# NJUVISION/PCGCv2

Hardware: AMD Instinct MI355X
Metric: encode+decode Mpoints/sec at fixed bpp (r3 ckpt), vox10 frame (higher is better)
Workload: dtype f32

## Files before the change

pcgcv2_amd/csrc/child_irn.hip:

```cpp
#include "child_kernels.h"

#define DECL_IRN_LAUNCH(NAME) int NAME(const int32_t* parent_nbr, int64_t n_parent, const float* in, int in_ld, const float* table, \
                                       int table_bytes, const IrnEpi& ep, hipStream_t s)
DECL_IRN_LAUNCH(pcgc_irn_child_a16); DECL_IRN_LAUNCH(pcgc_irn_child_b16);
DECL_IRN_LAUNCH(pcgc_irn_child_a32); DECL_IRN_LAUNCH(pcgc_irn_child_b32);

extern "C" int pcgc_irn_child_pass(const int32_t* parent_nbr, int64_t n_parent, int C, int pass, const float* in, int in_ld,
                                   const float* table, int64_t table_bytes, const float* b0, const float* b1, const float* b2,
                                   const float* x, int x_ld, float* out, int out_ld, void* stream) {
    CHILD_COMMON_CHECKS(in_ld)
    PCGC_REQUIRE(C == 16 || C == 32, "channels must be 16 or 32 (C = 64 blocks run on pcgc_irn_rows_pass through the level's own map)");
    PCGC_REQUIRE(pass == 1 || pass == 2, "pass must be 1 (A) or 2 (B)");
    PCGC_REQUIRE(out && b0 && b1 && (pass == 1 || (b2 && x)), "null argument");
    PCGC_REQUIRE((out_ld & 3) == 0 && (((uintptr_t)out) & 15) == 0 && (pass == 1 || ((x_ld & 3) == 0 && (((uintptr_t)x) & 15) == 0)),
                 "rows must be 16-byte aligned");
    PCGC_REQUIRE(pass == 2 || out_ld == C / 2, "pass A writes a dense [rows, C/2] tensor");
    hipStream_t s = S(stream);
    IrnEpi ep{b0, b1, b2, x, x_ld, out, out_ld};
    const int tb = (int)table_bytes;
    int rc;
    if (pass == 1) {
        PCGC_REQUIRE(table_bytes == (int64_t)(C == 16 ? 52 : 38) * (C / 16) * 1024, "pass A table size");
        rc = C == 16 ? pcgc_irn_child_a16(parent_nbr, n_parent, in, in_ld, table, tb, ep, s) : pcgc_irn_child_a32(parent_nbr, n_parent, in, in_ld, table, tb, ep, s);
    } else {
        PCGC_REQUIRE(table_bytes == (int64_t)(C == 16 ? 85 * 64 * 4 : 64 * 128 * 4), "pass B table size");
        rc = C == 16 ? pcgc_irn_child_b16(parent_nbr, n_parent, in, in_ld, table, tb, ep, s) : pcgc_irn_child_b32(parent_nbr, n_parent, in, in_ld, table, tb, ep, s);
    }
    if (rc) return rc;
    PCGC_CHECK_LAUNCH("irn_child_pass");
    return 0;
}

#ifdef PCGC_CHILD_TIMING
extern "C" int pcgc_child_timing_irn(unsigned long long* out8, int reset) {
    hipDeviceSynchronize();
    if (out8) hipMemcpyFromSymbol(out8, HIP_SYMBOL(g_child_dbg), 8 * sizeof(unsigned long long));
    if (reset) { unsigned long long z[8] = {0}; hipMemcpyToSymbol(HIP_SYMBOL(g_child_dbg), z, sizeof(z)); }
    return 0;
}
// ... 2 lines not shown
```

pcgcv2_amd/csrc/child_kernels.h:

```cpp
#pragma once
#include "pcgc_common.h"
#include "mfma_util.h"
#include <type_traits>

#ifdef PCGC_CHILD_TIMING
static __device__ unsigned long long g_child_dbg[8];
#define CHILD_T(var) const unsigned long long var = __builtin_amdgcn_s_memtime()
#define CHILD_TADD(slot, a, b) do { child_dbg[slot] += (b) - (a); } while (0)
#define CHILD_DBG_DECL unsigned long long child_dbg[8] = {0, 0, 0, 0, 0, 0, 0, 0};
#define CHILD_DBG_PARAM , unsigned long long (&child_dbg)[8]
#define CHILD_DBG_ARG , child_dbg
#define CHILD_TFLUSH do { if ((threadIdx.x & 63) == 0) { for (int q_ = 0; q_ < 8; ++q_) if (child_dbg[q_]) atomicAdd(&g_child_dbg[q_], child_dbg[q_]); } } while (0)
#define CHILD_TIMING_READER(NAME)                                                                                      \
    extern "C" int NAME(unsigned long long* out8, int reset) {                                                         \
        (void)hipDeviceSynchronize();                                                                                  \
        if (out8) (void)hipMemcpyFromSymbol(out8, HIP_SYMBOL(g_child_dbg), 8 * sizeof(unsigned long long));           \
        if (reset) { unsigned long long z[8] = {0}; (void)hipMemcpyToSymbol(HIP_SYMBOL(g_child_dbg), z, sizeof(z)); }  \
        return 0;                                                                                                      \
    }
#else
#define CHILD_T(var)
#define CHILD_TADD(slot, a, b)
#define CHILD_DBG_DECL
#define CHILD_DBG_PARAM
// ... 86 lines not shown
    static constexpr int tz(int t) { return CPT == 4 ? (t % TH) : (t % TH) >> 1; }
    static constexpr int ty(int t) { return (t % TH) & 1; }
    static constexpr bool active(int c, int t) {
        const int kz = cz_of(c) - tz(t);
        if (HZ >= 0 && tz(t) != HZ) return false;
        if (CPT == 4) {
            if (t < TH) return in02(kz);
            return kz == 1 && (cy_of(c) == 1 || cy_of(c) == 2) && (cx_of(c) == 1 || cx_of(c) == 2);
        }
        const int ky = cy_of(c) - ty(t);
        if (t < TH) return in02(kz) && in02(ky);
        return kz == 1 && ky == 1 && (cx_of(c) == 1 || cx_of(c) == 2);
    }
    static constexpr int N0 = CPT == 4 ? 48 : (CPT == 2 ? 36 : 27);
    static constexpr int frag(int c, int t) {
        const int kz = cz_of(c) - tz(t);
        if (CPT == 4) return t < TH ? kz * 16 + (c & 15) : N0 + (cy_of(c) - 1) * 2 + (cx_of(c) - 1);
        const int ky = cy_of(c) - ty(t);
        return t < TH ? (kz * 3 + ky) * 4 + cx_of(c) : N0 + (cx_of(c) - 1);
    }
    static constexpr bool uses_block(int, int) { return true; }
    static constexpr int frag_off(int c, int t, int cb) { return (frag(c, t) * NB + cb) * 64 * KS * 4; }
};
template <int C, int HZ = -1, bool T2_ = false>
struct PassB : HaloGeometry {
    static constexpr bool T2 = T2_;
    static_assert(!T2_ || C == 16, "the split layout exists for C = 16");
    static constexpr int Q = C / 4, NB = 1, ROWCHUNKS = Q / 2 , KS = Q / 4;
    static constexpr int CPT0 = 16 / (2 * Q) , T0 = 8 / CPT0, CPT1 = 16 / Q, T1 = 8 / CPT1, T = T0 + T1;
    static constexpr int Z_HALF = HZ;
    static_assert(HZ < 0 || CPT1 <= 2, "half units: no tile may hold children of both z halves");
    static constexpr bool HALF = false;
    static constexpr int kfirst(int t) { return t < T0 ? 0 : KS; }
    static constexpr int tile_z(int t) { return t < T0 ? ((t * CPT0) >> 2) & 1 : (((t - T0) * CPT1) >> 2) & 1; }
    static constexpr bool active(int c, int t) {
        if (HZ >= 0 && tile_z(t) != HZ) return false;
        if (t < T0) {
            if (CPT0 == 1) return (cell_reach(c) >> t) & 1;
            return in02(cz_of(c) - (t >> 1)) && in02(cy_of(c) - (t & 1));
        }
        const int u = t - T0;
        if (CPT1 == 2) return in02(cz_of(c) - (u >> 1)) && in02(cy_of(c) - (u & 1));
        return in02(cz_of(c) - u);
    }
    static constexpr int N0 = CPT0 == 1 ? 27 : 36;
    static constexpr int N1 = CPT1 == 2 ? 36 : 48;
    static constexpr int FRAG_W12 = N0 + N1;
    static constexpr int frag(int c, int t) {
        if (t < T0) {
            if (CPT0 == 1) return cell_k(c, t);
            return ((cz_of(c) - (t >> 1)) * 3 + (cy_of(c) - (t & 1))) * 4 + cx_of(c);
        }
        const int u = t - T0;
        if (CPT1 == 2) return N0 + ((cz_of(c) - (u >> 1)) * 3 + (cy_of(c) - (u & 1))) * 4 + cx_of(c);
        return N0 + (cz_of(c) - u) * 16 + (c & 15);
    }
    static constexpr bool uses_block(int, int) { return true; }
    static constexpr int frag_off(int c, int t, int cb) { return (frag(c, t) * NB + cb) * 64 * KS * 4; }
};

template <class V, class = void> struct child_t2_layout : std::false_type {};
template <class V> struct child_t2_layout<V, std::enable_if_t<V::T2>> : std::true_type {};

template <int I, int N, typename F>
__device__ __forceinline__ void static_for(F&& f) {
    if constexpr (I < N) {
        f(std::integral_constant<int, I>{});
        static_for<I + 1, N>(f);
    }
}

template <int KS> struct BFrag;
template <> struct BFrag<4> {
    f32x4 v;
    template <int OFF> __device__ __forceinline__ void load(unsigned base) { asm volatile("ds_read_b128 %0, %1 offset:%2" : "=v"(v) : "v"(base), "n"(OFF) : "memory"); }
    __device__ __forceinline__ void tie() { asm volatile("" : "+v"(v)); }
    __device__ __forceinline__ float get(int i) const { return v[i]; }
};
typedef float f32x2 __attribute__((ext_vector_type(2)));
template <> struct BFrag<2> {
    f32x2 v;
    template <int OFF> __device__ __forceinline__ void load(unsigned base) { asm volatile("ds_read_b64 %0, %1 offset:%2" : "=v"(v) : "v"(base), "n"(OFF) : "memory"); }
    __device__ __forceinline__ void tie() { asm volatile("" : "+v"(v)); }
    __device__ __forceinline__ float get(int i) const { return v[i]; }
};
template <> struct BFrag<1> {
// ... 27 lines not shown
    const int64_t l = (blockIdx.x >> 3) + (int64_t)(gridDim.x >> 3) * (wave + NW * i);
    const int64_t tile = (blockIdx.x & 7) * S + l;
    return (l < S && tile < ntiles) ? tile : -1;
}

template <int NW>
__device__ __forceinline__ void child_stage_table(const float* __restrict__ table, int table_bytes, unsigned char* lds_raw) {
    float4* tab = (float4*)lds_raw;
    for (int i = threadIdx.x; i < table_bytes / 16; i += NW * 64) tab[i] = ((const float4*)table)[i];
    __syncthreads();
}

struct ChildCells { int n; int c[64]; };
template <class V> constexpr ChildCells child_cells() {
    ChildCells L{};
    for (int c = 0; c < V::NCELLS; ++c) {
        bool used = false;
        for (int t = 0; t < V::T; ++t) used = used || V::active(c, t);
        if (used) L.c[L.n++] = c;
    }
    return L;
}

template <class V, int D, int MT>
__device__ __forceinline__ void child_tile_mainloop_mt(const int32_t* __restrict__ pnbr, int64_t n_p, int64_t p0,
                                                       const __amdgpu_buffer_rsrc_t& rs_in, int in_ld, const unsigned char* lds_raw,
                                                       float4* ring, f32x4 (&acc)[MT][V::T] CHILD_DBG_PARAM) {
    constexpr int NB = V::NB, T = V::T, KS = V::KS;
    static_assert(MT == 1 || MT == 2, "one or two M tiles per wave");
    static_assert((D & (D - 1)) == 0, "ring depth must be a power of two");
    static_assert((D - 1) * NB * MT < 64, "vmcnt is 6 bits");
    CHILD_T(t_tile0);
    const int lane = threadIdx.x & 63;
    const int mi = lane & 15, mq = lane >> 4;
    const int dma_r = lane >> 2;
    bool row_ok[MT];
#pragma unroll
    for (int m = 0; m < MT; ++m) row_ok[m] = p0 + 16 * m + dma_r < n_p;
    constexpr unsigned ABSENT = 0xF0000000u;
    unsigned rowb[MT][V::NMAP];
#pragma unroll
    for (int m = 0; m < MT; ++m)
#pragma unroll
        for (int kp = 0; kp < V::NMAP; ++kp) rowb[m][kp] = (unsigned)pnbr[(int64_t)kp * n_p + (row_ok[m] ? p0 + 16 * m + dma_r : 0)];
    const int f_a = (0x78 >> (2 * (mi >> 2))) & 3;
    const int dma_chunk = (lane & 3) ^ ((0x78 >> (2 * ((dma_r >> 2) & 3))) & 3);
    const bool chunk_ok = dma_chunk < V::ROWCHUNKS;
    const unsigned row_bytes = (unsigned)in_ld * 4u;
    asm volatile("s_waitcnt vmcnt(0)" ::: "memory");
#pragma unroll
    for (int m = 0; m < MT; ++m)
#pragma unroll
        for (int kp = 0; kp < V::NMAP; ++kp)
            rowb[m][kp] = (row_ok[m] && (int)rowb[m][kp] >= 0) ? rowb[m][kp] * ((unsigned)V::ROW_MUL * row_bytes) : ABSENT;
    constexpr bool T2 = child_t2_layout<V>::value;
    const unsigned lane_off = chunk_ok ? (unsigned)dma_chunk * (T2 ? 64u : 16u) : ABSENT;
    CHILD_T(t_loop0);

    constexpr ChildCells CL = child_cells<V>();
    constexpr int NC = CL.n;
    auto issue = [&](auto ii) {
        constexpr int i = decltype(ii)::value, c = CL.c[i];
        float4* dst = ring + (i & (D - 1)) * (MT * NB * 64);
#pragma unroll
        for (int m = 0; m < MT; ++m) {
            unsigned voff = rowb[m][V::kp(c)] + (T2 ? (unsigned)((V::child(c) >> 2) * 128 + (V::child(c) & 3) * 16) : (unsigned)V::child(c) * row_bytes) + lane_off +
                            (unsigned)V::byte_off(c);
            if constexpr (V::ROWCHUNKS < 4) voff = chunk_ok ? voff : 0xFFFFFFF0u;
#pragma unroll
            for (int cb = 0; cb < NB; ++cb)
                __builtin_amdgcn_raw_ptr_buffer_load_lds(rs_in, (lds_void_ptr)(dst + (m * NB + cb) * 64), 16, (int)(voff + cb * 64), 0, 0, 0);
        }
        asm volatile("" ::: "memory");
    };

#pragma unroll
    for (int m = 0; m < MT; ++m)
#pragma unroll
        for (int t = 0; t < T; ++t) acc[m][t] = (f32x4){0.f, 0.f, 0.f, 0.f};
    unsigned tab_lane;
    if constexpr (V::HALF) tab_lane = (unsigned)(uintptr_t)(lds_void_ptr)(lds_raw + V::lane_table_off(mi, mq));
    else tab_lane = (unsigned)(uintptr_t)(lds_void_ptr)((const float*)lds_raw + lane * KS);
    unsigned a_addr[4];
#pragma unroll
    for (int jj = 0; jj < 4; ++jj) a_addr[jj] = (unsigned)(uintptr_t)(lds_void_ptr)((const float*)ring + (mi * 4 + (jj ^ f_a)) * 4 + mq);
    constexpr unsigned ksteps_used = [] { unsigned m = 0; for (int t = 0; t < T; ++t) for (int j = 0; j < KS; ++j) m |= 1u << (V::kfirst(t) + j); return m; }();

    static_assert(NB * T <= 32, "all B fragments of a cell are held in registers at once");
    static_for<0, (D < NC ? D : NC)>(issue);
    static_for<0, NC>([&](auto ii) {
        constexpr int i = decltype(ii)::value, c = CL.c[i];
        constexpr int younger = (NC - 1 - i) < (D - 1) ? (NC - 1 - i) : (D - 1);
        wait_vmcnt<younger * NB * MT>();
        float a[MT][NB][4];
        BFrag<KS> b[NB][T];
        static_for<0, NB>([&](auto icb) {
            constexpr int cb = decltype(icb)::value;
            static_for<0, MT>([&](auto im) {
                constexpr int m = decltype(im)::value;
                static_for<0, 4>([&](auto ij) {
                    constexpr int jj = decltype(ij)::value;
                    if constexpr ((ksteps_used >> jj) & 1)
                        a[m][cb][jj] = lds_ld32_off<(((i & (D - 1)) * MT + m) * NB + cb) * 1024>(a_addr[jj]);
                });
            });
            static_for<0, T>([&](auto it) {
                constexpr int t = decltype(it)::value;
                if constexpr (V::active(c, t) && V::uses_block(t, cb)) {
                    constexpr int off = V::frag_off(c, t, cb);
                    if constexpr (off < 65536) b[cb][t].template load<off>(tab_lane);
                    else b[cb][t].template load<off - 65536>(tab_lane + 65536);
                }
            });
        });
        asm volatile("s_waitcnt lgkmcnt(0)" ::: "memory");
        static_for<0, NB>([&](auto icb) {
            constexpr int cb = decltype(icb)::value;
            static_for<0, MT>([&](auto im) {
                static_for<0, 4>([&](auto ij) {
                    constexpr int jj = decltype(ij)::value;
                    if constexpr ((ksteps_used >> jj) & 1) lds_tie(a[decltype(im)::value][cb][jj]);
                });
            });
            static_for<0, T>([&](auto it) {
                constexpr int t = decltype(it)::value;
                if constexpr (V::active(c, t) && V::uses_block(t, cb)) b[cb][t].tie();
            });
        });
        if constexpr (i + D < NC) issue(std::integral_constant<int, i + D>{});
        static_for<0, NB>([&](auto icb) {
            constexpr int cb = decltype(icb)::value;
            static_for<0, 4>([&](auto ij) {
                constexpr int jj = decltype(ij)::value;
                static_for<0, T>([&](auto it) {
                    constexpr int t = decltype(it)::value;
                    if constexpr (V::active(c, t) && V::uses_block(t, cb) && jj >= V::kfirst(t) && jj < V::kfirst(t) + KS) {
                        static_for<0, MT>([&](auto im) {
                            constexpr int m = decltype(im)::value;
                            acc[m][t] = __builtin_amdgcn_mfma_f32_16x16x4f32(a[m][cb][jj], b[cb][t].get(jj - V::kfirst(t)), acc[m][t], 0, 0, 0);
                        });
                    }
                });
            });
        });
    });
#ifdef PCGC_CHILD_TIMING
    asm volatile("s_nop 0" : "+v"(acc[0][0]));
    CHILD_T(t_loop1);
    CHILD_TADD(0, t_tile0, t_loop0);
    CHILD_TADD(1, t_loop0, t_loop1);
    CHILD_TADD(3, 0ull, 1ull);
#endif
}

template <class V, int D>
__device__ __forceinline__ void child_tile_mainloop(const int32_t* __restrict__ pnbr, int64_t n_p, int64_t p0,
                                                    const __amdgpu_buffer_rsrc_t& rs_in, int in_ld, const unsigned char* lds_raw,
                                                    float4* ring, f32x4 (&acc)[V::T] CHILD_DBG_PARAM) {
    child_tile_mainloop_mt<V, D, 1>(pnbr, n_p, p0, rs_in, in_ld, lds_raw, ring, reinterpret_cast<f32x4 (&)[1][V::T]>(acc) CHILD_DBG_ARG);
}

__device__ __forceinline__ void wave_lds_sync() {
    __builtin_amdgcn_fence(__ATOMIC_RELEASE, "wavefront");
    __builtin_amdgcn_wave_barrier();
    __builtin_amdgcn_fence(__ATOMIC_ACQUIRE, "wavefront");
}

template <int W, int ROWS>
struct ChildResidual { float4 x[(ROWS * (W / 4) + 63) / 64]; };
template <int W, int ROWS>
__device__ __forceinline__ void child_flush_prefetch(ChildResidual<W, ROWS>& rr, int64_t row0, int64_t rows_total, const float* __restrict__ res,
                                                     int res_ld, int lane, int half = -1) {
    constexpr int C4 = W / 4, N = (ROWS * C4 + 63) / 64;
    if (!res) return;
#pragma unroll
    for (int it = 0; it < N; ++it) {
        const int i = lane + 64 * it, lr = i / C4, c4 = i % C4;
        const int64_t row = row0 + lr;
        const bool ok = i < ROWS * C4 && row < rows_total && !(half >= 0 && ((lr >> 2) & 1) != half);
        rr.x[it] = ok ? *(const float4*)(res + row * res_ld + 4 * c4) : make_float4(0.f, 0.f, 0.f, 0.f);
    }
}
template <int W, int ROWS>
__device__ __forceinline__ void child_flush(const float* scratch, const ChildResidual<W, ROWS>& rr, bool has_res, int64_t row0, int64_t rows_total,
                                            float* __restrict__ out, int out_ld, int relu, int lane, int half = -1) {
    constexpr int C4 = W / 4, N = (ROWS * C4 + 63) / 64;
    ChildResidual<W, ROWS> xr = rr;
    if (has_res) {
#pragma unroll
        for (int it = 0; it < N; ++it) asm volatile("" : "+v"(xr.x[it].x), "+v"(xr.x[it].y), "+v"(xr.x[it].z), "+v"(xr.x[it].w));
    }
#pragma unroll
    for (int it = 0; it < N; ++it) {
        const int i = lane + 64 * it, lr = i / C4, c4 = i % C4;
        const int64_t row = row0 + lr;
        if (i >= ROWS * C4 || row >= rows_total || (half >= 0 && ((lr >> 2) & 1) != half)) continue;
        float4 v = ((const float4*)scratch)[i];
        if (has_res) {
            const float4 x = xr.x[it];
            v.x = v.x + x.x; v.y = v.y + x.y; v.z = v.z + x.z; v.w = v.w + x.w;
        }
        if (relu) { v.x = fmaxf(v.x, 0.0f); v.y = fmaxf(v.y, 0.0f); v.z = fmaxf(v.z, 0.0f); v.w = fmaxf(v.w, 0.0f); }
        *(float4*)(out + row * out_ld + 4 * c4) = v;
// ... 182 lines not shown
                child_flush<W, CH>(scratch, 8 * p0 + h * CH, 8 * n_p, ep.out, W, 0, lane, HZ);
                wave_lds_sync();
            }
        }
    };
    const int64_t nunits = (SPLIT ? 2 : 1) * ((n_p + 16 * MT - 1) / (16 * MT));
    for (int i = 0;; ++i) {
        const int64_t u = child_tile<NW>(i, wave, nunits);
        if (u < 0) break;
        CHILD_T(t_it0);
        if constexpr (SPLIT) {
            if (u & 1) unit(child_type_tag<PassA<C, 1>>{}, (u >> 1) * (16 * MT));
            else unit(child_type_tag<PassA<C, 0>>{}, (u >> 1) * (16 * MT));
        } else {
            unit(child_type_tag<V>{}, u * (16 * MT));
        }
#ifdef PCGC_CHILD_TIMING
        { CHILD_T(t_dr0); asm volatile("s_waitcnt vmcnt(0)" ::: "memory"); CHILD_T(t_it1); CHILD_TADD(5, t_dr0, t_it1); CHILD_TADD(4, t_it0, t_it1); }
#endif
    }
    CHILD_TFLUSH;
}

template <int C, int NW, int D, bool SPLIT = false, int MT = 1, bool T2 = false>
__global__ void __launch_bounds__(NW * 64)
k_child_irn_b(const int32_t* __restrict__ pnbr, int64_t n_p, const float* __restrict__ in , int in_ld,
              const float* __restrict__ table, int table_bytes, IrnEpi ep) {
    using V = PassB<C, -1, T2>;
    constexpr int Q = V::Q, H = 2 * Q, KQ = Q / 4, T0 = V::T0, T1 = V::T1, CPT0 = V::CPT0, CPT1 = V::CPT1;
    constexpr int CH = ((128 * Q + 64 * C) * 4 <= D * 1024 * MT) ? 64 : 32, MQC = CH / 32;
    constexpr int NEEDF4 = (128 * Q + CH * C) / 4;
    constexpr int RINGF4 = (D * 64 * MT > NEEDF4) ? D * 64 * MT : NEEDF4;
    CHILD_KERNEL_PROLOGUE(V, NW, D, RINGF4)
    float* us = (float*)ring;
    float* stage = us + 128 * Q;
    float w12[KQ];
#pragma unroll
    for (int jj = 0; jj < KQ; ++jj) w12[jj] = ((const float*)lds_raw)[V::FRAG_W12 * frag_floats<V>() + lane * KQ + jj];
    const int c1 = mi % Q, sub1 = mi / Q, c0 = mi % H, sub0 = mi / H;
    const float b11 = ep.b1[c1], b01 = ep.b0[c0], b12 = mi < H ? ep.b2[mi] : 0.0f;
    auto unit = [&](auto tag, const int64_t pu) {
        using VV = typename decltype(tag)::type;
        constexpr int HZ = VV::Z_HALF;
        f32x4 acc[MT][VV::T];
        child_tile_mainloop_mt<VV, D, MT>(pnbr, n_p, pu, rs_in, in_ld, lds_raw, ring, acc CHILD_DBG_ARG);
#pragma unroll
        for (int m = 0; m < MT; ++m) {
        const int64_t p0 = pu + 16 * m;
        if (m > 0 && p0 >= n_p) break;
        ChildResidual<C, CH> rr;
        child_flush_prefetch<C, CH>(rr, 8 * p0, 8 * n_p, ep.x, ep.x_ld, lane, HZ);
        {
#pragma unroll
            for (int u = 0; u < T1; ++u) {
                if (HZ >= 0 && VV::tile_z(T0 + u) != HZ) continue;
#pragma unroll
                for (int r = 0; r < 4; ++r) us[(8 * (4 * mq + r) + u * CPT1 + sub1) * Q + c1] = fmaxf(acc[m][T0 + u][r] + b11, 0.0f);
            }
        }
        wave_lds_sync();
        {
#pragma unroll
            for (int h = 0; h < 128 / CH; ++h) {
                if (h > 0) child_flush_prefetch<C, CH>(rr, 8 * p0 + h * CH, 8 * n_p, ep.x, ep.x_ld, lane, HZ);
                if (mq / MQC == h) {
#pragma unroll
                    for (int t = 0; t < T0; ++t) {
                        if (HZ >= 0 && VV::tile_z(t) != HZ) continue;
                        const int j = t * CPT0 + sub0;
#pragma unroll
                        for (int r = 0; r < 4; ++r) stage[(8 * (4 * (mq % MQC) + r) + j) * C + c0] = acc[m][t][r] + b01;
                    }
                }
                float au[CH / 16][KQ];
// ... 7 lines not shown
                    d[gg] = (f32x4){0.f, 0.f, 0.f, 0.f};
#pragma unroll
                    for (int jj = 0; jj < KQ; ++jj) d[gg] = __builtin_amdgcn_mfma_f32_16x16x4f32(au[gg][jj], w12[jj], d[gg], 0, 0, 0);
                }
                if (mi < H) {
#pragma unroll
                    for (int gg = 0; gg < CH / 16; ++gg)
#pragma unroll
                        for (int r = 0; r < 4; ++r) stage[(16 * gg + 4 * mq + r) * C + H + mi] = d[gg][r] + b12;
                }
                wave_lds_sync();
                child_flush<C, CH>(stage, rr, ep.x != nullptr, 8 * p0 + h * CH, 8 * n_p, ep.out, ep.out_ld, 0, lane, HZ);
                wave_lds_sync();
            }
        }
        }
    };
    const int64_t nunits = (SPLIT ? 2 : 1) * ((n_p + 16 * MT - 1) / (16 * MT));
    for (int i = 0;; ++i) {
        const int64_t u = child_tile<NW>(i, wave, nunits);
        if (u < 0) break;
        CHILD_T(t_it0);
        if constexpr (SPLIT) {
            if (u & 1) unit(child_type_tag<PassB<C, 1, T2>>{}, (u >> 1) * (16 * MT));
            else unit(child_type_tag<PassB<C, 0, T2>>{}, (u >> 1) * (16 * MT));
        } else {
            unit(child_type_tag<V>{}, u * (16 * MT));
        }
#ifdef PCGC_CHILD_TIMING
        { CHILD_T(t_dr0); asm volatile("s_waitcnt vmcnt(0)" ::: "memory"); CHILD_T(t_it1); CHILD_TADD(5, t_dr0, t_it1); CHILD_TADD(4, t_it0, t_it1); }
#endif
    }
    CHILD_TFLUSH;
}

struct ChildLdsGrant { size_t bytes[16] = {0}; };
template <typename K>
int child_lds_limit(K kern, size_t lds, ChildLdsGrant& granted) {
    if (lds > 160 * 1024) { pcgc_set_error("child kernel: %zu bytes of LDS needed", lds); return -2; }
    int dev = 0;
    (void)hipGetDevice(&dev);
    size_t& g = granted.bytes[dev & 15];
    if (lds > 48 * 1024 && lds > g) {
        hipError_t e = hipFuncSetAttribute((const void*)kern, hipFuncAttributeMaxDynamicSharedMemorySize, (int)lds);
        if (e != hipSuccess) { pcgc_set_error("child kernel: cannot raise the LDS limit to %zu: %s", lds, hipGetErrorString(e)); return -1; }
        g = lds;
    }
    return 0;
// ... 37 lines not shown
    CHILD_LAUNCH_EX((k_child_conv<NB, NT, NW, D, true, 1, false>), NW, D * NB * 1024, ep, 1, 2);
}
template <int NB, int NW, int D, int MT = 1, int WPC = 16>
int launch_child_cls(const int32_t* pnbr, int64_t n_p, const float* in, int in_ld, const float* table, int table_bytes,
                     const ChildEpi& ep, hipStream_t s) {
    const size_t lds = (size_t)table_bytes + (size_t)NW * (D * NB * 1024 * MT);
    auto kern = k_child_cls<NB, NW, D, MT>;
    static ChildLdsGrant granted;
    if (int rc = child_lds_limit(kern, lds, granted)) return rc;
    const int64_t units = (n_p + 16 * MT - 1) / (16 * MT);
    hipLaunchKernelGGL(kern, dim3(child_grid_units(units, NW, lds, WPC)), dim3(NW * 64), lds, s, pnbr, n_p, in, in_ld, table, table_bytes, ep);
    return 0;
}
template <int C, int NW, int D, int MT = 1>
int launch_child_irn_a(const int32_t* pnbr, int64_t n_p, const float* in, int in_ld, const float* table, int table_bytes,
                       const IrnEpi& ep, hipStream_t s) {
    CHILD_LAUNCH_EX((k_child_irn_a<C, NW, D, false, MT>), NW, D * (C / 16) * 1024 * MT, ep, MT, 1);
}
template <int C, int NW, int D>
int launch_child_irn_a_split(const int32_t* pnbr, int64_t n_p, const float* in, int in_ld, const float* table, int table_bytes,
                             const IrnEpi& ep, hipStream_t s) {
    CHILD_LAUNCH_SPLIT((k_child_irn_a<C, NW, D, true>), NW, D * (C / 16) * 1024, ep);
}
template <int C, int NW, int D, int MT = 1, bool T2 = false>
int launch_child_irn_b(const int32_t* pnbr, int64_t n_p, const float* in, int in_ld, const float* table, int table_bytes,
                       const IrnEpi& ep, hipStream_t s) {
    constexpr int Q = C / 4, CH = ((128 * Q + 64 * C) * 4 <= D * 1024 * MT) ? 64 : 32;
    constexpr int need = (128 * Q + CH * C) * 4;
    constexpr int ringb = (D * 1024 * MT > need) ? D * 1024 * MT : need;
    CHILD_LAUNCH_EX((k_child_irn_b<C, NW, D, false, MT, T2>), NW, ringb, ep, MT, 1);
}
template <int C, int NW, int D>
int launch_child_irn_b_split(const int32_t* pnbr, int64_t n_p, const float* in, int in_ld, const float* table, int table_bytes,
                             const IrnEpi& ep, hipStream_t s) {
    constexpr int Q = C / 4, CH = ((128 * Q + 64 * C) * 4 <= D * 1024) ? 64 : 32;
    constexpr int need = (128 * Q + CH * C) * 4;
    constexpr int ringb = (D * 1024 > need) ? D * 1024 : need;
    CHILD_LAUNCH_SPLIT((k_child_irn_b<C, NW, D, true>), NW, ringb, ep);
}

}

#define CHILD_COMMON_CHECKS(ROWS_LD)                                                                                           \
    PCGC_REQUIRE(parent_nbr && in && table, "null argument");                                                                  \
    PCGC_REQUIRE(((ROWS_LD) & 3) == 0 && (((uintptr_t)in | (uintptr_t)table) & 15) == 0, "unaligned input");                 \
    PCGC_REQUIRE(8 * n_parent * (int64_t)(ROWS_LD) * 4 < (int64_t)0xF0000000, "tensor too large for 32-bit buffer offsets"); \
    PCGC_REQUIRE(table_bytes % 16 == 0, "table size");                                                                         \
    if (n_parent == 0) return 0;
```

pcgcv2_amd/csrc/child_q4.h:

```cpp
#pragma once
#include "child_kernels.h"

namespace {

struct Q4Group {
    int cell, child, kind;
    int k;
    bool first, last;
    bool fin;
};
struct Q4Sched {
    int n;
    Q4Group g[232];
    int vm_wait[232];
    int pend[232];
};
constexpr int Q4_PASS_A = 0, Q4_CLS = 1;
template <int KIND, int MT, int D = 2>
constexpr Q4Sched q4_sched() {
    Q4Sched S{};
    for (int c = 0; c < 64; ++c) {
        const int n0 = S.n;
        if (KIND == Q4_CLS) {
            for (int h = 0; h < 2; ++h)
// ... 18 lines not shown
        if (G.first && G.cell + D < 64) { ops += 4 * MT; gather_end[G.cell + D] = ops; }
        S.pend[n] = pending;
        ops += pending;
        pending = (KIND == Q4_PASS_A && ((G.kind == 1) || G.fin) && (G.child & 3) == 3) ? 4 * MT : 0;
    }
    return S;
}

typedef unsigned u32x4 __attribute__((ext_vector_type(4)));
__device__ __forceinline__ void q4_store(const f32x4& v, const __amdgpu_buffer_rsrc_t& rs, unsigned voff) {
    u32x4 u = {__float_as_uint(v[0]), __float_as_uint(v[1]), __float_as_uint(v[2]), __float_as_uint(v[3])};
#ifndef Q4_STORE_AUX
#define Q4_STORE_AUX 0
#endif
    __builtin_amdgcn_raw_buffer_store_b128(u, rs, (int)voff, 0, Q4_STORE_AUX);
}

template <int KIND, int NW, int MT, int D = 2>
__global__ void __launch_bounds__(NW * 64)
k_child_q4(const int32_t* __restrict__ pnbr, int64_t n_p, const float* __restrict__ in, int in_ld,
           const float* __restrict__ table, int table_bytes, IrnEpi ep) {
    constexpr int TP = 64 * MT, SLOT_F4 = MT * 256;
    constexpr Q4Sched S = q4_sched<KIND, MT, D>();
    constexpr int NACC = KIND == Q4_CLS ? 2 : 8, OUT_ROW_BYTES = KIND == Q4_CLS ? 4 : 32;
    extern __shared__ __attribute__((aligned(16))) unsigned char lds_raw[];
    const int lane = threadIdx.x & 63;
    const int wave = __builtin_amdgcn_readfirstlane(threadIdx.x >> 6);
    float4* ring = (float4*)(lds_raw + table_bytes) + wave * (D * SLOT_F4);
    child_stage_table<NW>(table, table_bytes, lds_raw);
    const __amdgpu_buffer_rsrc_t rs_in = __builtin_amdgcn_make_buffer_rsrc((void*)in, 0, (int)(8 * n_p * in_ld * 4), 0x00020000);
    const __amdgpu_buffer_rsrc_t rs_out = __builtin_amdgcn_make_buffer_rsrc((void*)ep.out, 0, (int)(8 * n_p * OUT_ROW_BYTES), 0x00020000);
    const int co = lane & 3;
    float b00[4], b10[4];
#pragma unroll
    for (int r = 0; r < 4; ++r) { b00[r] = KIND == Q4_CLS ? (ep.b0 ? ep.b0[0] : 0.0f) : ep.b0[r]; b10[r] = KIND == Q4_CLS ? 0.0f : ep.b1[r]; }
    const unsigned tab_lane = (unsigned)(uintptr_t)(lds_void_ptr)((const float*)lds_raw + co * 16);
    const unsigned a_row = (unsigned)(uintptr_t)(lds_void_ptr)((const float*)ring + lane * 16 + (((lane >> 2) & 3) << 2));
    const unsigned row_bytes = (unsigned)in_ld * 4u;
    const unsigned lane_off = (unsigned)(((lane & 3) ^ ((lane >> 4) & 3)) * 16);
    constexpr unsigned ABSENT = 0xF0000000u;
    const int64_t ntiles = (n_p + TP - 1) / TP;

    for (int it = 0;; ++it) {
#ifdef Q4_EXP_TILE_ORDER
        int64_t tile;
        {
// ... 6 lines not shown
        const int64_t tile = child_tile<NW>(it, wave, ntiles);
#endif
        if (tile < 0) break;
        const int64_t p_base = tile * TP;
        unsigned rowb[MT][27];
        bool ok[MT];
#pragma unroll
        for (int m = 0; m < MT; ++m) {
            const int64_t rho = p_base + 64 * m + 16 * (lane & 3) + (lane >> 2);
            ok[m] = rho < n_p;
#pragma unroll
            for (int kp = 0; kp < 27; ++kp) rowb[m][kp] = (unsigned)pnbr[(int64_t)kp * n_p + (ok[m] ? rho : 0)];
        }
        asm volatile("s_waitcnt vmcnt(0)" ::: "memory");
#pragma unroll
        for (int m = 0; m < MT; ++m)
#pragma unroll
            for (int kp = 0; kp < 27; ++kp)
#ifdef Q4_KO_GATHER
                rowb[m][kp] = ((int)rowb[m][kp] == 0x7FFFFFF1) ? rowb[m][kp] * (8u * row_bytes) : ABSENT;
#else
                rowb[m][kp] = (ok[m] && (int)rowb[m][kp] >= 0) ? rowb[m][kp] * (8u * row_bytes) : ABSENT;
#endif
        auto ovq = [&](int m) { return (unsigned)((p_base + 64 * m + (lane & ~3)) * 256 + (lane & 3) * 16); };
#ifdef Q4_KO_STORE
        f32x4 sink = (f32x4){0.f, 0.f, 0.f, 0.f};
#endif

        f32x4 acc0[MT][NACC], c1[MT][KIND == Q4_CLS ? 1 : 4];
#pragma unroll
        for (int m = 0; m < MT; ++m)
#pragma unroll
            for (int j = 0; j < NACC; ++j) acc0[m][j] = (f32x4){0.f, 0.f, 0.f, 0.f};
        f32x4 a[MT][4], b[2][4];

        auto gather = [&](auto ic) {
            constexpr int c = decltype(ic)::value, kp = cell_kp(c), ch = cell_child(c), slot = c % D;
            const unsigned cell_off = (unsigned)ch * row_bytes + lane_off;
#pragma unroll
            for (int m = 0; m < MT; ++m) {
                const int rb = (int)rowb[m][kp];
                const unsigned v0 = (unsigned)__builtin_amdgcn_update_dpp(0, rb, 0x00, 0xF, 0xF, true) + cell_off;
                const unsigned v1 = (unsigned)__builtin_amdgcn_update_dpp(0, rb, 0x55, 0xF, 0xF, true) + cell_off;
                const unsigned v2 = (unsigned)__builtin_amdgcn_update_dpp(0, rb, 0xAA, 0xF, 0xF, true) + cell_off;
                const unsigned v3 = (unsigned)__builtin_amdgcn_update_dpp(0, rb, 0xFF, 0xF, 0xF, true) + cell_off;
                float4* dst = ring + slot * SLOT_F4 + m * 256;
                __builtin_amdgcn_raw_ptr_buffer_load_lds(rs_in, (lds_void_ptr)(dst), 16, (int)v0, 0, 0, 0);
// ... 35 lines not shown
                static_for<0, MT>([&](auto im) {
                    constexpr int m = decltype(im)::value;
                    f32x4 V[4], W[4];
#pragma unroll
                    for (int k = 0; k < 4; ++k) {
                        if constexpr (G.kind == 1) V[k] = c1[m][k];
                        else {
#pragma unroll
                            for (int r = 0; r < 4; ++r) V[k][r] = fmaxf(acc0[m][4 * h + k][r] + b00[r], 0.0f);
                        }
                    }
#pragma unroll
                    for (int r = 0; r < 4; ++r) W[r] = (f32x4){0.f, 0.f, 0.f, 0.f};
#pragma unroll
                    for (int k = 0; k < 4; ++k)
#pragma unroll
                        for (int r = 0; r < 4; ++r) W[r] = __builtin_amdgcn_mfma_f32_4x4x1f32(V[k][r], onehot[k], W[r], 0, 0, 0);
#pragma unroll
                    for (int t = 0; t < 4; ++t) {
                        const f32x4 v = {W[0][t], W[1][t], W[2][t], W[3][t]};
#ifdef Q4_KO_STORE
                        sink = sink + v;
#else
                        q4_store(v, rs_out, ovq(m) + (unsigned)(t * 256 + h * 128 + (G.kind == 1 ? 64 : 0)));
#endif
                    }
                });
            }
        };

        using I0 = std::integral_constant<int, 0>;
        static_for<0, D>(gather);
        wait_vmcnt<4 * MT * (D - 1)>();
        load_b(I0{}, I0{});
        static_for<0, 4>([&](auto ie) { load_a(I0{}, ie); });

        static_for<0, S.n>([&](auto in_) {
            constexpr int n = decltype(in_)::value, cur = n & 1;
            constexpr Q4Group G = S.g[n];
            constexpr bool has_next = n + 1 < S.n, next_cell = G.cell + 1 < 64;
            if constexpr (G.first) wait_lgkmcnt<3 * MT>(); else wait_lgkmcnt<0>();
            static_for<0, 4>([&](auto ie) { lds_tie(b[cur][decltype(ie)::value]); });
            if constexpr (G.first) static_for<0, MT>([&](auto im) { lds_tie(a[decltype(im)::value][0]); });
            if constexpr (has_next) load_b(std::integral_constant<int, has_next ? n + 1 : n>{}, std::integral_constant<int, cur ^ 1>{});
            if constexpr (G.last && next_cell) wait_vmcnt<S.vm_wait[n]>();
            if constexpr (G.kind == 1) static_for<0, MT>([&](auto im) { c1[decltype(im)::value][G.child & 3] = (f32x4){0.f, 0.f, 0.f, 0.f}; });
            static_for<0, 4>([&](auto ie) {
// ... 68 lines not shown
```

pcgcv2_amd/csrc/child_q4.hip:

```cpp
#include "child_q4.h"

extern "C" int pcgc_irn_child_q4(const int32_t* parent_nbr, int64_t n_parent, int C, int pass, const float* in, int in_ld,
                                 const float* table, int64_t table_bytes, const float* b0, const float* b1, const float* b2,
                                 const float* x, int x_ld, float* out, int out_ld, void* stream) {
    CHILD_COMMON_CHECKS(in_ld)
    PCGC_REQUIRE(C == 16, "the quad-block kernels serve C = 16");
    PCGC_REQUIRE(pass == 1 || pass == 2, "pass must be 1 (A) or 2 (B)");
    PCGC_REQUIRE(out && b0 && b1 && (pass == 1 || (b2 && x)), "null argument");
    PCGC_REQUIRE((out_ld & 3) == 0 && (((uintptr_t)out) & 15) == 0 && (pass == 1 || ((x_ld & 3) == 0 && (((uintptr_t)x) & 15) == 0)),
                 "rows must be 16-byte aligned");
    hipStream_t s = S(stream);
    IrnEpi ep{b0, b1, b2, x, x_ld, out, out_ld};
    int rc;
    if (pass == 1) {
        PCGC_REQUIRE(out_ld == C / 2, "pass A writes a dense [rows, C/2] tensor");
        PCGC_REQUIRE(table_bytes == 28 * 64 * 4, "pass A table size");
        rc = launch_child_q4<Q4_PASS_A, 8, 2>(parent_nbr, n_parent, in, in_ld, table, (int)table_bytes, ep, s);
    } else {
        PCGC_REQUIRE(in_ld == C / 2, "pass B reads the dense [rows, C/2] tensor of pass A");
        PCGC_REQUIRE(table_bytes == 85 * 64 * 4, "pass B table size");
        rc = launch_child_irn_b<16, 16, 8, 1, true>(parent_nbr, n_parent, in, in_ld, table, (int)table_bytes, ep, s);
    }
    if (rc) return rc;
    PCGC_CHECK_LAUNCH("irn_child_q4");
    return 0;
}

extern "C" int pcgc_cls_child_q4(const int32_t* parent_nbr, int64_t n_parent, const float* in, int Cin, int in_ld,
                                 const float* table, int64_t table_bytes, const float* bias, float* out, void* stream) {
    CHILD_COMMON_CHECKS(in_ld)
    PCGC_REQUIRE(Cin == 16, "the quad-block classification head serves C = 16");
    PCGC_REQUIRE(out && (((uintptr_t)out) & 15) == 0, "the output must be 16-byte aligned");
    PCGC_REQUIRE(table_bytes == 96 * 64 * 4, "cls table size");
    IrnEpi ep{bias, nullptr, nullptr, nullptr, 0, out, 1};
    const int rc = launch_child_q4<Q4_CLS, 8, 2>(parent_nbr, n_parent, in, in_ld, table, (int)table_bytes, ep, S(stream));
    if (rc) return rc;
    PCGC_CHECK_LAUNCH("cls_child_q4");
    return 0;
}
```

pcgcv2_amd/dispatch.py:

```python
from collections import namedtuple

from . import ops

LIMIT = 0xF0000000

Rule = namedtuple('Rule', 'op shape level rows_min rows_max switch family kernel why')
INF = 1 << 62

TABLE = (
    Rule('conv3', ((16, 16), (32, 32), (16, 1), (32, 1), (64, 1)), 'children', 8192, INF, 'CHILD_MFMA', 'child',
         'k_child_conv<1,1> / k_child_conv<2,2,split> / k_child_cls<NB>; 16->1 with CHILD_Q4: k_child_q4<cls> (quad-block 4x4x1 MFMA)',
         'halo gather through the parent map, packed-N fp32 MFMA: conv 16->16 436 -> 259 us on 2.05 M rows, cls 16->1 209 -> 85 (quad-block form: 83)'),
    Rule('conv3', ((1, 16),), None, 0, INF, 'UNIT_INPUT_CONV', 'unit', 'k_conv_unit<16> / k_conv_unit_coarse<16>',
         'all-ones occupancy input (x.has_unit_features()): sum of kernel slices over the present offsets, no feature gathers: 88 -> 55 us'),
    Rule('conv3', ((32, 32),), None, 'ROWS_CONV_MIN', INF, 'ROWS_CONV', 'rows', 'k_rows_conv<2,2>',
         'LDS-resident fragment table, one wave per 16-row tile: 34 vs 51 us at 1-18 k rows, 127 vs 159 at 256 k'),
    Rule('conv3', ((64, 64),), None, 'PACKED_CONV64_MIN', INF, 'PACKED_CONV64', 'packed', 'k_conv_packed64',
         'present rows packed per workgroup tile and offset, accumulators in LDS, B fragments in registers: conv2 (71 k rows) 215 -> 118 us, conv0 (150 k) 335 -> 306 (profiles/r04_conv_packed.md)'),
    Rule('conv3', None, None, 0, INF, None, 'gather', 'pcgc_conv_gather (see GATHER below)', 'every other shape / size'),
    Rule('irn', (16, 32), 'children', 8192, INF, 'CHILD_MFMA', 'child',
         'k_child_irn_a<C> + k_child_irn_b<C> (C = 32: half units); C = 16 with CHILD_Q4: k_child_q4<pass A> (quad-block 4x4x1 MFMA) + k_child_irn_b<16, T2 gather>',
         'packed-N MFMA passes through the parent map: C = 16 212/170 -> 118/102 us on 2.05 M rows (quad-block pass A: 97/110), C = 32 174/130 -> 100/81 on 570 k'),
    Rule('irn', (64,), None, 'ROWS_IRN64_MIN', INF, 'ROWS_IRN64', 'rows64', 'k_rows_irn_a64<.., RowsPassA64H> + k_rows_irn_b64',
         "through the level's own map, plain or children level (the decoder's 64 -> 64 conv has built it): 65 vs 135 us per block at 1-18 k rows, 103 vs 198 at 71 k; "
         'on the 150 k-row children level 171 vs 197 us for the parent-map form (removed in round 5)'),
    Rule('irn', (32,), None, 'ROWS_Q4_MIN', 'ROWS_IRN32_MAX+1', 'ROWS_Q4', 'rows32q4', 'k_rows_q4_a32 + k_rows_q4_b32',
         'quad-block form (4x4x1 fp32 MFMA, lane = row, no zero column: issued / algorithmic 3.9 -> 2.1 in pass A): 120 -> 88 us per block at 256 k rows; '
         'below ~150 k rows the 64-row tiles are one round of lone waves and the packed-N kernels stay ahead (40 vs 46 us at 71 k)'),
    Rule('irn', (32,), None, 'ROWS_IRN32_MIN', 'ROWS_IRN32_MAX+1', 'ROWS_IRN32', 'rows32', 'k_rows_irn_a32 + k_rows_irn_b32',
         'plain level: 47 vs 74 us per block at 49 k rows, 119 vs 127 at 256 k'),
    Rule('irn', (16, 32, 64), None, 0, INF, 'FUSE_IRN', 'valu', 'k_irn_a_split<C> + k_irn_b_split<C> (C = 16, 32), k_irn_a<64,16> + k_irn_b<64,16>',
         'two fused gather passes on the VALU, 16-row tiles: levels below 1024 rows, children levels below 8192'),
    Rule('irn', None, None, 0, INF, None, 'unfused', 'five MinkowskiConvolution calls + fused epilogues', 'any other channel count'),
    Rule('down', ((16, 32), (32, 64), (64, 32)), None, 'ROWS_DOWN_MIN', INF, 'ROWS_DOWN', 'rows_down', 'k_rows_down<NB,NT>',
         'tile = 16 coarse rows walking the 8 child offsets: 121 -> ~65 us for the three down convs of a vox10 frame (rows = COARSE rows)'),
    Rule('down', None, None, 0, INF, None, 'gather', 'pcgc_conv_gather, K = 8', 'other shapes / tiny levels'),
    Rule('conv1', None, None, 0, INF, None, 'gather', 'pcgc_conv_gather, K = 1 (k_conv_gather_valu)', 'k1 convs outside fused blocks'),
    Rule('prune', (8, 16, 32, 64), None, 0, INF, 'ONE_SWEEP_PRUNE', 'select', 'k_topk_init + 3 x k_topk_hist + k_topk_select',
         'thresholds by radix select, then ONE scan writes coordinates, survivor rows and a rank bitmap: 10 -> 5 launches per decoder stage'),
    Rule('prune', None, None, 0, INF, None, 'mask', 'pcgc_topk_mask(_segments) + pcgc_mask_scan + pcgc_compact_*', 'byte mask + int32 prefix per row'),
    Rule('up', None, None, 0, INF, None, 'up2', 'k_conv_up2_mfma<64,32> / <32,16>, k_conv_up2_rows otherwise', 'generative transpose, one kernel per shape'),
)

GATHER_IMPL_NAMES = {0: 'k_conv_gather_valu', 2: 'k_conv_gather_mfma', 6: 'k_conv_gather_split (row-split)'}
# ... 75 lines not shown
```

Measured before the change: 144.8.

## Prefetch residual rows inside pass-B mainloop and drop the T2 split layout

For C = 16 single-tile unsplit pass B, the residual rows are now loaded with buffer loads issued inside the gather mainloop at a hook point, with the vmcnt waits adjusted so the loads overlap with the MFMA work instead of being fetched after the loop. The T2 interleaved pass-A output layout is removed: the q4 pass A store offsets change back to a plain layout and q4 pass B now calls the regular b16 launcher. A 32-bit offset guard and a vmcnt static check are added. This trades extra registers held across the mainloop for hidden residual load latency.

```diff
diff --git a/pcgcv2_amd/csrc/child_irn.hip b/pcgcv2_amd/csrc/child_irn.hip
--- a/pcgcv2_amd/csrc/child_irn.hip
+++ b/pcgcv2_amd/csrc/child_irn.hip
@@ -15,6 +15,7 @@
     PCGC_REQUIRE((out_ld & 3) == 0 && (((uintptr_t)out) & 15) == 0 && (pass == 1 || ((x_ld & 3) == 0 && (((uintptr_t)x) & 15) == 0)),
                  "rows must be 16-byte aligned");
     PCGC_REQUIRE(pass == 2 || out_ld == C / 2, "pass A writes a dense [rows, C/2] tensor");
+    PCGC_REQUIRE(pass == 1 || 8 * n_parent * (int64_t)x_ld * 4 < (int64_t)0xF0000000, "residual too large for 32-bit buffer offsets");
     hipStream_t s = S(stream);
     IrnEpi ep{b0, b1, b2, x, x_ld, out, out_ld};
     const int tb = (int)table_bytes;
diff --git a/pcgcv2_amd/csrc/child_kernels.h b/pcgcv2_amd/csrc/child_kernels.h
--- a/pcgcv2_amd/csrc/child_kernels.h
+++ b/pcgcv2_amd/csrc/child_kernels.h
@@ -132,10 +132,8 @@
     static constexpr bool uses_block(int, int) { return true; }
     static constexpr int frag_off(int c, int t, int cb) { return (frag(c, t) * NB + cb) * 64 * KS * 4; }
 };
-template <int C, int HZ = -1, bool T2_ = false>
+template <int C, int HZ = -1>
 struct PassB : HaloGeometry {
-    static constexpr bool T2 = T2_;
-    static_assert(!T2_ || C == 16, "the split layout exists for C = 16");
     static constexpr int Q = C / 4, NB = 1, ROWCHUNKS = Q / 2 , KS = Q / 4;
     static constexpr int CPT0 = 16 / (2 * Q) , T0 = 8 / CPT0, CPT1 = 16 / Q, T1 = 8 / CPT1, T = T0 + T1;
     static constexpr int Z_HALF = HZ;
@@ -169,9 +167,6 @@
     static constexpr int frag_off(int c, int t, int cb) { return (frag(c, t) * NB + cb) * 64 * KS * 4; }
 };
 
-template <class V, class = void> struct child_t2_layout : std::false_type {};
-template <class V> struct child_t2_layout<V, std::enable_if_t<V::T2>> : std::true_type {};
-
 template <int I, int N, typename F>
 __device__ __forceinline__ void static_for(F&& f) {
     if constexpr (I < N) {
@@ -245,14 +240,14 @@
     return L;
 }
 
-template <class V, int D, int MT>
-__device__ __forceinline__ void child_tile_mainloop_mt(const int32_t* __restrict__ pnbr, int64_t n_p, int64_t p0,
-                                                       const __amdgpu_buffer_rsrc_t& rs_in, int in_ld, const unsigned char* lds_raw,
-                                                       float4* ring, f32x4 (&acc)[MT][V::T] CHILD_DBG_PARAM) {
+template <class V, int D, int MT, int PRE, class PF>
+__device__ __forceinline__ void child_tile_mainloop_pre(const int32_t* __restrict__ pnbr, int64_t n_p, int64_t p0,
+                                                        const __amdgpu_buffer_rsrc_t& rs_in, int in_ld, const unsigned char* lds_raw,
+                                                        float4* ring, f32x4 (&acc)[MT][V::T], PF&& pre CHILD_DBG_PARAM) {
     constexpr int NB = V::NB, T = V::T, KS = V::KS;
     static_assert(MT == 1 || MT == 2, "one or two M tiles per wave");
     static_assert((D & (D - 1)) == 0, "ring depth must be a power of two");
-    static_assert((D - 1) * NB * MT < 64, "vmcnt is 6 bits");
+    static_assert(PRE >= 0 && (D - 1) * NB * MT + PRE < 64, "vmcnt is 6 bits");
     CHILD_T(t_tile0);
     const int lane = threadIdx.x & 63;
     const int mi = lane & 15, mq = lane >> 4;
@@ -276,8 +271,7 @@
 #pragma unroll
         for (int kp = 0; kp < V::NMAP; ++kp)
             rowb[m][kp] = (row_ok[m] && (int)rowb[m][kp] >= 0) ? rowb[m][kp] * ((unsigned)V::ROW_MUL * row_bytes) : ABSENT;
-    constexpr bool T2 = child_t2_layout<V>::value;
-    const unsigned lane_off = chunk_ok ? (unsigned)dma_chunk * (T2 ? 64u : 16u) : ABSENT;
+    const unsigned lane_off = chunk_ok ? (unsigned)dma_chunk * 16u : ABSENT;
     CHILD_T(t_loop0);
 
     constexpr ChildCells CL = child_cells<V>();
@@ -287,8 +281,7 @@
         float4* dst = ring + (i & (D - 1)) * (MT * NB * 64);
 #pragma unroll
         for (int m = 0; m < MT; ++m) {
-            unsigned voff = rowb[m][V::kp(c)] + (T2 ? (unsigned)((V::child(c) >> 2) * 128 + (V::child(c) & 3) * 16) : (unsigned)V::child(c) * row_bytes) + lane_off +
-                            (unsigned)V::byte_off(c);
+            unsigned voff = rowb[m][V::kp(c)] + (unsigned)V::child(c) * row_bytes + lane_off + (unsigned)V::byte_off(c);
             if constexpr (V::ROWCHUNKS < 4) voff = chunk_ok ? voff : 0xFFFFFFF0u;
 #pragma unroll
             for (int cb = 0; cb < NB; ++cb)
@@ -310,11 +303,13 @@
     constexpr unsigned ksteps_used = [] { unsigned m = 0; for (int t = 0; t < T; ++t) for (int j = 0; j < KS; ++j) m |= 1u << (V::kfirst(t) + j); return m; }();
 
     static_assert(NB * T <= 32, "all B fragments of a cell are held in registers at once");
+    constexpr int HOOK = NC > D ? NC - 1 - D : -1;
     static_for<0, (D < NC ? D : NC)>(issue);
+    if constexpr (PRE > 0 && HOOK < 0) pre();
     static_for<0, NC>([&](auto ii) {
         constexpr int i = decltype(ii)::value, c = CL.c[i];
         constexpr int younger = (NC - 1 - i) < (D - 1) ? (NC - 1 - i) : (D - 1);
-        wait_vmcnt<younger * NB * MT>();
+        wait_vmcnt<younger * NB * MT + ((PRE > 0 && i > HOOK) ? PRE : 0)>();
         float a[MT][NB][4];
         BFrag<KS> b[NB][T];
         static_for<0, NB>([&](auto icb) {
@@ -351,6 +346,7 @@
             });
         });
         if constexpr (i + D < NC) issue(std::integral_constant<int, i + D>{});
+        if constexpr (PRE > 0 && i == HOOK) pre();
         static_for<0, NB>([&](auto icb) {
             constexpr int cb = decltype(icb)::value;
             static_for<0, 4>([&](auto ij) {
@@ -376,6 +372,13 @@
 #endif
 }
 
+template <class V, int D, int MT>
+__device__ __forceinline__ void child_tile_mainloop_mt(const int32_t* __restrict__ pnbr, int64_t n_p, int64_t p0,
+                                                       const __amdgpu_buffer_rsrc_t& rs_in, int in_ld, const unsigned char* lds_raw,
+                                                       float4* ring, f32x4 (&acc)[MT][V::T] CHILD_DBG_PARAM) {
+    child_tile_mainloop_pre<V, D, MT, 0>(pnbr, n_p, p0, rs_in, in_ld, lds_raw, ring, acc, [] {} CHILD_DBG_ARG);
+}
+
 template <class V, int D>
 __device__ __forceinline__ void child_tile_mainloop(const int32_t* __restrict__ pnbr, int64_t n_p, int64_t p0,
                                                     const __amdgpu_buffer_rsrc_t& rs_in, int in_ld, const unsigned char* lds_raw,
@@ -402,6 +405,19 @@
         const int64_t row = row0 + lr;
         const bool ok = i < ROWS * C4 && row < rows_total && !(half >= 0 && ((lr >> 2) & 1) != half);
         rr.x[it] = ok ? *(const float4*)(res + row * res_ld + 4 * c4) : make_float4(0.f, 0.f, 0.f, 0.f);
+    }
+}
+typedef unsigned child_u32x4 __attribute__((ext_vector_type(4)));
+template <int W, int ROWS>
+__device__ __forceinline__ void child_flush_prefetch_buf(ChildResidual<W, ROWS>& rr, int64_t row0, const __amdgpu_buffer_rsrc_t& rs_res,
+                                                         int res_ld, int lane) {
+    constexpr int C4 = W / 4, N = ROWS * C4 / 64;
+    static_assert(ROWS * C4 % 64 == 0, "whole instructions only");
+#pragma unroll
+    for (int it = 0; it < N; ++it) {
+        const int i = lane + 64 * it, lr = i / C4, c4 = i % C4;
+        const child_u32x4 u = __builtin_amdgcn_raw_buffer_load_b128(rs_res, (int)(((unsigned)(row0 + lr) * (unsigned)res_ld + 4u * c4) * 4u), 0, 0);
+        rr.x[it] = make_float4(__uint_as_float(u[0]), __uint_as_float(u[1]), __uint_as_float(u[2]), __uint_as_float(u[3]));
     }
 }
 template <int W, int ROWS>
@@ -630,11 +646,11 @@
     CHILD_TFLUSH;
 }
 
-template <int C, int NW, int D, bool SPLIT = false, int MT = 1, bool T2 = false>
+template <int C, int NW, int D, bool SPLIT = false, int MT = 1>
 __global__ void __launch_bounds__(NW * 64)
 k_child_irn_b(const int32_t* __restrict__ pnbr, int64_t n_p, const float* __restrict__ in , int in_ld,
               const float* __restrict__ table, int table_bytes, IrnEpi ep) {
-    using V = PassB<C, -1, T2>;
+    using V = PassB<C, -1>;
     constexpr int Q = V::Q, H = 2 * Q, KQ = Q / 4, T0 = V::T0, T1 = V::T1, CPT0 = V::CPT0, CPT1 = V::CPT1;
     constexpr int CH = ((128 * Q + 64 * C) * 4 <= D * 1024 * MT) ? 64 : 32, MQC = CH / 32;
     constexpr int NEEDF4 = (128 * Q + CH * C) / 4;
@@ -647,17 +663,23 @@
     for (int jj = 0; jj < KQ; ++jj) w12[jj] = ((const float*)lds_raw)[V::FRAG_W12 * frag_floats<V>() + lane * KQ + jj];
     const int c1 = mi % Q, sub1 = mi / Q, c0 = mi % H, sub0 = mi / H;
     const float b11 = ep.b1[c1], b01 = ep.b0[c0], b12 = mi < H ? ep.b2[mi] : 0.0f;
+    constexpr bool EARLY_RES = C == 16 && MT == 1 && !SPLIT;
+    constexpr int NRES = EARLY_RES ? CH * (C / 4) / 64 : 0;
+    const __amdgpu_buffer_rsrc_t rs_x = __builtin_amdgcn_make_buffer_rsrc((void*)ep.x, 0, EARLY_RES ? (int)(8 * n_p * ep.x_ld * 4) : 0, 0x00020000);
     auto unit = [&](auto tag, const int64_t pu) {
         using VV = typename decltype(tag)::type;
         constexpr int HZ = VV::Z_HALF;
         f32x4 acc[MT][VV::T];
-        child_tile_mainloop_mt<VV, D, MT>(pnbr, n_p, pu, rs_in, in_ld, lds_raw, ring, acc CHILD_DBG_ARG);
+        ChildResidual<C, CH> rr;
+        if constexpr (EARLY_RES)
+            child_tile_mainloop_pre<VV, D, MT, NRES>(pnbr, n_p, pu, rs_in, in_ld, lds_raw, ring, acc,
+                                                     [&] { child_flush_prefetch_buf<C, CH>(rr, 8 * pu, rs_x, ep.x_ld, lane); } CHILD_DBG_ARG);
+        else child_tile_mainloop_mt<VV, D, MT>(pnbr, n_p, pu, rs_in, in_ld, lds_raw, ring, acc CHILD_DBG_ARG);
 #pragma unroll
         for (int m = 0; m < MT; ++m) {
         const int64_t p0 = pu + 16 * m;
         if (m > 0 && p0 >= n_p) break;
-        ChildResidual<C, CH> rr;
-        child_flush_prefetch<C, CH>(rr, 8 * p0, 8 * n_p, ep.x, ep.x_ld, lane, HZ);
+        if constexpr (!EARLY_RES) child_flush_prefetch<C, CH>(rr, 8 * p0, 8 * n_p, ep.x, ep.x_ld, lane, HZ);
         {
 #pragma unroll
             for (int u = 0; u < T1; ++u) {
@@ -711,8 +733,8 @@
         if (u < 0) break;
         CHILD_T(t_it0);
         if constexpr (SPLIT) {
-            if (u & 1) unit(child_type_tag<PassB<C, 1, T2>>{}, (u >> 1) * (16 * MT));
-            else unit(child_type_tag<PassB<C, 0, T2>>{}, (u >> 1) * (16 * MT));
+            if (u & 1) unit(child_type_tag<PassB<C, 1>>{}, (u >> 1) * (16 * MT));
+            else unit(child_type_tag<PassB<C, 0>>{}, (u >> 1) * (16 * MT));
         } else {
             unit(child_type_tag<V>{}, u * (16 * MT));
         }
@@ -796,13 +818,13 @@
                              const IrnEpi& ep, hipStream_t s) {
     CHILD_LAUNCH_SPLIT((k_child_irn_a<C, NW, D, true>), NW, D * (C / 16) * 1024, ep);
 }
-template <int C, int NW, int D, int MT = 1, bool T2 = false>
+template <int C, int NW, int D, int MT = 1>
 int launch_child_irn_b(const int32_t* pnbr, int64_t n_p, const float* in, int in_ld, const float* table, int table_bytes,
                        const IrnEpi& ep, hipStream_t s) {
     constexpr int Q = C / 4, CH = ((128 * Q + 64 * C) * 4 <= D * 1024 * MT) ? 64 : 32;
     constexpr int need = (128 * Q + CH * C) * 4;
     constexpr int ringb = (D * 1024 * MT > need) ? D * 1024 * MT : need;
-    CHILD_LAUNCH_EX((k_child_irn_b<C, NW, D, false, MT, T2>), NW, ringb, ep, MT, 1);
+    CHILD_LAUNCH_EX((k_child_irn_b<C, NW, D, false, MT>), NW, ringb, ep, MT, 1);
 }
 template <int C, int NW, int D>
 int launch_child_irn_b_split(const int32_t* pnbr, int64_t n_p, const float* in, int in_ld, const float* table, int table_bytes,
diff --git a/pcgcv2_amd/csrc/child_q4.h b/pcgcv2_amd/csrc/child_q4.h
--- a/pcgcv2_amd/csrc/child_q4.h
+++ b/pcgcv2_amd/csrc/child_q4.h
@@ -64,6 +64,7 @@
            const float* __restrict__ table, int table_bytes, IrnEpi ep) {
     constexpr int TP = 64 * MT, SLOT_F4 = MT * 256;
     constexpr Q4Sched S = q4_sched<KIND, MT, D>();
+    static_assert([] { int w = 0; for (int n = 0; n < S.n; ++n) w = S.vm_wait[n] > w ? S.vm_wait[n] : w; return w; }() < 64, "vmcnt is 6 bits");
     constexpr int NACC = KIND == Q4_CLS ? 2 : 8, OUT_ROW_BYTES = KIND == Q4_CLS ? 4 : 32;
     extern __shared__ __attribute__((aligned(16))) unsigned char lds_raw[];
     const int lane = threadIdx.x & 63;
@@ -116,7 +117,7 @@
 #else
                 rowb[m][kp] = (ok[m] && (int)rowb[m][kp] >= 0) ? rowb[m][kp] * (8u * row_bytes) : ABSENT;
 #endif
-        auto ovq = [&](int m) { return (unsigned)((p_base + 64 * m + (lane & ~3)) * 256 + (lane & 3) * 16); };
+        auto ovq = [&](int m) { return (unsigned)((p_base + 64 * m + (lane & ~3)) * 256 + (lane & 3) * 32); };
 #ifdef Q4_KO_STORE
         f32x4 sink = (f32x4){0.f, 0.f, 0.f, 0.f};
 #endif
@@ -198,7 +199,7 @@
 #ifdef Q4_KO_STORE
                         sink = sink + v;
 #else
-                        q4_store(v, rs_out, ovq(m) + (unsigned)(t * 256 + h * 128 + (G.kind == 1 ? 64 : 0)));
+                        q4_store(v, rs_out, ovq(m) + (unsigned)(t * 256 + h * 128 + (G.kind == 1 ? 16 : 0)));
 #endif
                     }
                 });
diff --git a/pcgcv2_amd/csrc/child_q4.hip b/pcgcv2_amd/csrc/child_q4.hip
--- a/pcgcv2_amd/csrc/child_q4.hip
+++ b/pcgcv2_amd/csrc/child_q4.hip
@@ -1,5 +1,7 @@
 #include "child_q4.h"
 
+int pcgc_irn_child_b16(const int32_t* parent_nbr, int64_t n_parent, const float* in, int in_ld, const float* table, int table_bytes,
+                       const IrnEpi& ep, hipStream_t s);
 extern "C" int pcgc_irn_child_q4(const int32_t* parent_nbr, int64_t n_parent, int C, int pass, const float* in, int in_ld,
                                  const float* table, int64_t table_bytes, const float* b0, const float* b1, const float* b2,
                                  const float* x, int x_ld, float* out, int out_ld, void* stream) {
@@ -19,7 +21,8 @@
     } else {
         PCGC_REQUIRE(in_ld == C / 2, "pass B reads the dense [rows, C/2] tensor of pass A");
         PCGC_REQUIRE(table_bytes == 85 * 64 * 4, "pass B table size");
-        rc = launch_child_irn_b<16, 16, 8, 1, true>(parent_nbr, n_parent, in, in_ld, table, (int)table_bytes, ep, s);
+        PCGC_REQUIRE(8 * n_parent * (int64_t)x_ld * 4 < (int64_t)0xF0000000, "residual too large for 32-bit buffer offsets");
+        rc = pcgc_irn_child_b16(parent_nbr, n_parent, in, in_ld, table, (int)table_bytes, ep, s);
     }
     if (rc) return rc;
     PCGC_CHECK_LAUNCH("irn_child_q4");
diff --git a/pcgcv2_amd/dispatch.py b/pcgcv2_amd/dispatch.py
--- a/pcgcv2_amd/dispatch.py
+++ b/pcgcv2_amd/dispatch.py
@@ -19,7 +19,7 @@
          'present rows packed per workgroup tile and offset, accumulators in LDS, B fragments in registers: conv2 (71 k rows) 215 -> 118 us, conv0 (150 k) 335 -> 306 (profiles/r04_conv_packed.md)'),
     Rule('conv3', None, None, 0, INF, None, 'gather', 'pcgc_conv_gather (see GATHER below)', 'every other shape / size'),
     Rule('irn', (16, 32), 'children', 8192, INF, 'CHILD_MFMA', 'child',
-         'k_child_irn_a<C> + k_child_irn_b<C> (C = 32: half units); C = 16 with CHILD_Q4: k_child_q4<pass A> (quad-block 4x4x1 MFMA) + k_child_irn_b<16, T2 gather>',
+         'k_child_irn_a<C> + k_child_irn_b<C> (C = 32: half units); C = 16 with CHILD_Q4: k_child_q4<pass A> (quad-block 4x4x1 MFMA) + k_child_irn_b<16>',
          'packed-N MFMA passes through the parent map: C = 16 212/170 -> 118/102 us on 2.05 M rows (quad-block pass A: 97/110), C = 32 174/130 -> 100/81 on 570 k'),
     Rule('irn', (64,), None, 'ROWS_IRN64_MIN', INF, 'ROWS_IRN64', 'rows64', 'k_rows_irn_a64<.., RowsPassA64H> + k_rows_irn_b64',
          "through the level's own map, plain or children level (the decoder's 64 -> 64 conv has built it): 65 vs 135 us per block at 1-18 k rows, 103 vs 198 at 71 k; "
```

After: 144.1 (median of 2 runs). Within noise of the previous version (-0.5%).
